# stephaneguindon/phyml

Hardware: AMD Instinct MI355X
Metric: M partial-lk site-updates/sec on full-tree Lk() (higher is better)
Workload: dtype f64

## Files before the change

### include/phyhip.h

```cpp
#ifndef PHYHIP_H
#define PHYHIP_H

#ifdef __cplusplus
extern "C" {
#endif

#define PHYHIP_SUCCESS                         0
#define PHYHIP_ERROR_GENERAL                  (-1)
#define PHYHIP_ERROR_OUT_OF_MEMORY            (-2)
#define PHYHIP_ERROR_UNIDENTIFIED_EXCEPTION   (-3)
#define PHYHIP_ERROR_UNINITIALIZED_INSTANCE   (-4)
#define PHYHIP_ERROR_OUT_OF_RANGE             (-5)
#define PHYHIP_ERROR_NO_RESOURCE              (-6)
#define PHYHIP_ERROR_NO_IMPLEMENTATION        (-7)
#define PHYHIP_ERROR_FLOATING_POINT           (-8)

#define PHYHIP_OP_NONE (-1)

#define PHYHIP_FLAG_SHARDED (1L << 40)
#define PHYHIP_UNIQUE_ID_BYTES 128
#define PHYHIP_FLAG_CLASS_AXIS (1L << 41)
#define PHYHIP_FLAG_GENERIC_LOOP (1L << 42)

typedef struct
// ... 175 lines not shown
int phyhip_get_resident_stats(int instance, long long out[8]);

int phyhip_get_big_resident_stats(int instance, long long out[4]);

int phyhip_set_virtual_buffers(int instance, int minOperations);

int phyhip_get_virtual_stats(int instance, long long out[4]);

int phyhip_get_deferred_stats(int instance, long long out[4]);

int phyhip_set_chained_buffers(int instance, int minOperations);

int phyhip_get_chained_stats(int instance, long long out[4]);

int phyhip_get_record_stats(int instance, long long out[12]);


typedef struct { int destination, child1, child2; } phyhip_parsimony_operation;

int phyhip_set_parsimony(int instance, int general, const int *stepMatrix);
int phyhip_update_partial_parsimony(int instance, const phyhip_parsimony_operation *ops, int count);
int phyhip_calculate_edge_parsimony(int instance, int buffer1, int buffer2, long long *outParsimony);
int phyhip_get_site_parsimony(int instance, int *outSitePars);
int phyhip_get_partial_parsimony(int instance, int bufferIndex, int *outUi, int *outPars, int *outPPars );
int phyhip_profile_read_parsimony(int instance, double *outKernelMs, int *outLaunches, double *outPatternUpdates);

typedef struct { int child1, child2, subtree; } phyhip_parsimony_candidate;
int phyhip_calculate_regraft_parsimony(int instance, const phyhip_parsimony_candidate *candidates, int count, int keepCandidate,
                                       long long *outParsimony );
int phyhip_get_regraft_site_parsimony(int instance, int *outSitePars );
// ... 60 lines not shown
```

### phyml_amd/capi.py

```python
from __future__ import annotations

import ctypes as C
import os

import numpy as np

_HERE = os.path.dirname(os.path.abspath(__file__))
LIB_DIR = os.environ.get("PHYHIP_LIBDIR") or os.path.join(_HERE, "lib")
LIB_PATH = os.path.join(LIB_DIR, "libphyhip.so")


class PhyhipError(RuntimeError):
    code = None


class Operation(C.Structure):
    _fields_ = [("destinationPartials", C.c_int), ("destinationScaleWrite", C.c_int), ("destinationScaleRead", C.c_int),
                ("child1Partials", C.c_int), ("child1TransitionMatrix", C.c_int),
                ("child2Partials", C.c_int), ("child2TransitionMatrix", C.c_int)]


class RegraftCandidate(C.Structure):
    _fields_ = [("child1Partials", C.c_int), ("child2Partials", C.c_int), ("subtreePartials", C.c_int), ("flags", C.c_int),
                ("child1Length", C.c_double), ("child2Length", C.c_double), ("subtreeLength", C.c_double)]
# ... 20 lines not shown
                ("flags", C.c_long), ("computeUnits", C.c_int), ("globalMemBytes", C.c_longlong)]


SYMBOLS = [
    "phyhip_create_instance", "phyhip_finalize_instance", "phyhip_get_last_error", "phyhip_set_tip_partials",
    "phyhip_set_tip_states", "phyhip_set_tip_partials_at_pattern", "phyhip_set_partials", "phyhip_set_pattern_weights", "phyhip_set_category_rates",
    "phyhip_set_category_weights", "phyhip_set_state_frequencies", "phyhip_set_eigen_decomposition",
    "phyhip_set_phyml_options", "phyhip_set_invariant_sites", "phyhip_update_transition_matrices",
    "phyhip_set_transition_matrix", "phyhip_get_transition_matrix", "phyhip_update_partials",
    "phyhip_calculate_edge_log_likelihoods", "phyhip_calculate_edge_log_likelihoods_device",
    "phyhip_get_site_log_likelihoods", "phyhip_get_site_outputs", "phyhip_get_partials", "phyhip_get_scale_factors",
    "phyhip_set_scale_factors", "phyhip_get_numerical_warning", "phyhip_update_eigen_lr",
    "phyhip_calculate_eigen_lnl_dlnl", "phyhip_calculate_eigen_lnl", "phyhip_get_dot_prod", "phyhip_set_stream",
    "phyhip_synchronize", "phyhip_profile", "phyhip_profile_read", "phyhip_calculate_mixture_log_likelihood",
    "phyhip_calculate_mixture_eigen_lnl_dlnl", "phyhip_comm_get_unique_id", "phyhip_comm_init_rank", "phyhip_comm_size",
    "phyhip_get_shard_range", "phyhip_profile_read_kernel", "phyhip_profile_read_collective", "phyhip_profile_read_traffic", "phyhip_profile_read_eigen", "phyhip_get_resident_stats", "phyhip_get_big_resident_stats", "phyhip_set_virtual_buffers", "phyhip_get_virtual_stats", "phyhip_get_deferred_stats", "phyhip_set_chained_buffers", "phyhip_get_chained_stats", "phyhip_get_record_stats", "phyhip_calculate_class_mixture_log_likelihood",
    "phyhip_calculate_class_mixture_eigen_lnl_dlnl", "phyhip_get_class_scale_factors", "phyhip_set_mixture_invariant_sites",
    "phyhip_calculate_edge_site_outputs_exact", "phyhip_calculate_node_state_posteriors", "phyhip_profile_read_node_posteriors",
    "phyhip_calculate_pairwise_ml_distances", "phyhip_set_pairwise_work_space", "phyhip_profile_read_pairwise",
    "phyhip_set_support_site_log_likelihoods", "phyhip_calculate_sh_support", "phyhip_get_support_alias_table", "phyhip_profile_read_support",
    "phyhip_set_parsimony", "phyhip_update_partial_parsimony", "phyhip_calculate_edge_parsimony", "phyhip_get_site_parsimony",
    "phyhip_get_partial_parsimony", "phyhip_profile_read_parsimony",
    "phyhip_calculate_regraft_parsimony", "phyhip_get_regraft_site_parsimony", "phyhip_get_regraft_partial_parsimony",
    "phyhip_profile_read_regraft_parsimony",
    "phyhip_optimise_edge_length", "phyhip_profile_read_edge_length",
    "phyhip_calculate_regraft_log_likelihoods", "phyhip_get_regraft_partials", "phyhip_get_regraft_transition_matrix",
    "phyhip_set_regraft_work_space", "phyhip_profile_read_regraft",
    "phyhip_calculate_mixture_regraft_log_likelihoods", "phyhip_get_mixture_regraft_partials",
    "phyhip_get_mixture_regraft_transition_matrix", "phyhip_set_mixture_regraft_work_space", "phyhip_profile_read_mixture_regraft",
    "phyhip_optimise_triples", "phyhip_get_triple_partials", "phyhip_set_triple_work_space", "phyhip_profile_read_triples",
]
# ... 68 lines not shown
def comm_get_unique_id() -> bytes:
    buf = C.create_string_buffer(UNIQUE_ID_BYTES)
    _chk(load().phyhip_comm_get_unique_id(buf))
    return buf.raw


def load():
    global _lib
    if _lib is None:
        if not os.path.exists(LIB_PATH):
            raise PhyhipError(f"{LIB_PATH} not built: run __graft_entry__.build() (hipcc --offload-arch=gfx950)")
        L = C.CDLL(LIB_PATH)
        L.phyhip_get_last_error.restype = C.c_char_p
        _lib = L
    return _lib


def _chk(rc):
    if rc < 0:
        e = PhyhipError(f"phyhip error {rc}: {load().phyhip_get_last_error().decode()}")
        e.code = rc
        raise e
    return rc


def _f64(a):
    return np.ascontiguousarray(a, dtype=np.float64)


def _ptr(a):
# ... 443 lines not shown
        return tuple(int(v) for v in out)

    def set_chained_buffers(self, min_operations):
        _chk(self.L.phyhip_set_chained_buffers(self.id, int(min_operations)))

    def chained_stats(self):
        out = (C.c_longlong * 4)()
        _chk(self.L.phyhip_get_chained_stats(self.id, out))
        return tuple(int(v) for v in out)

    def record_stats(self):
        out = (C.c_longlong * 12)()
        _chk(self.L.phyhip_get_record_stats(self.id, out))
        return tuple(int(v) for v in out)

    def profile_read_eigen(self):
        a = C.c_double(0); an = C.c_int(0); b = C.c_double(0); bn = C.c_int(0)
        _chk(self.L.phyhip_profile_read_eigen(self.id, C.byref(a), C.byref(an), C.byref(b), C.byref(bn)))
        return (a.value, an.value), (b.value, bn.value)

    def profile_read_collective(self):
        ms = C.c_double(0); n = C.c_int(0); r = C.c_int(0)
        _chk(self.L.phyhip_profile_read_collective(self.id, C.byref(ms), C.byref(n), C.byref(r)))
        return ms.value, n.value, r.value

    def profile_read_kernel(self):
        buf = C.create_string_buffer(128)
        _chk(self.L.phyhip_profile_read_kernel(self.id, buf, 128))
        return buf.value.decode()

# ... 58 lines not shown
```

### phyml_amd/csrc/phyhip.hip

```cpp
#include "phyhip_host.hpp"
#include "phyhip_side.hpp"

namespace phyhip_host
{

int fail(int code, const char *fmt, ...)
{
  char    buf[512];
  va_list ap;
  va_start(ap, fmt);
  vsnprintf(buf, sizeof buf, fmt, ap);
  va_end(ap);
  g_err = buf;
  return code;
}

}

using namespace phyhip_host;

extern "C" {

const char *phyhip_get_last_error(void) { return g_err.c_str(); }

// ... 204 lines not shown
    HIPCHK(hipMalloc((void **)&I->d_afrag, fb));
    HIPCHK(hipMemset(I->d_afrag, 0, fb));
    const long long ntiles = I->Ppad / (16 / aa_cb(I->C));
    const long long cus    = prop.multiProcessorCount > 0 ? prop.multiProcessorCount : 256;
    I->aa_nw = (int)std::min<long long>(kAaMaxCons, std::max<long long>(1, (ntiles + cus - 1) / cus));
    if (const char *e = diag_env("PHYHIP_AA_NW")) { const int v = atoi(e); if (v >= 1 && v <= kAaMaxCons) I->aa_nw = v; }
    I->aa_d2 = false;
    if (const char *e = diag_env("PHYHIP_AA_D2")) I->aa_d2 = atoi(e) != 0 && I->aa_nw <= kAaMaxConsD2;
    I->aa_nt = 1;
    if (const char *e = diag_env("PHYHIP_AA_NT")) { const int v = atoi(e); if (v == 1 || v == 2) I->aa_nt = v; }
    if (I->aa_nt == 2) I->aa_nw = std::min(I->aa_nw, 2 * kAaMaxCons2);
    I->grid_aa = (int)((ntiles + I->aa_nw - 1) / I->aa_nw);
  }
  HIPCHK(hipMalloc((void **)&I->d_tipcodes, (size_t)I->tips * I->Ppad));
  HIPCHK(hipMemset(I->d_tipcodes, 0, (size_t)I->tips * I->Ppad));
  if (I->perm)
  {
    HIPCHK(hipMalloc((void **)&I->d_tipmasks, (size_t)I->tips * I->Ppad * sizeof(uint32_t)));
    HIPCHK(hipMemset(I->d_tipmasks, 0, (size_t)I->tips * I->Ppad * sizeof(uint32_t)));
  }
  HIPCHK(hipMalloc((void **)&I->d_masks, 256 * sizeof(uint32_t)));
  HIPCHK(hipMalloc((void **)&I->d_pmats, (size_t)I->nmat_all * I->C * I->S * I->S * sizeof(double)));
  HIPCHK(hipMemset(I->d_pmats, 0, (size_t)I->nmat_all * I->C * I->S * I->S * sizeof(double)));
  HIPCHK(hipMalloc((void **)&I->d_wght, I->P * sizeof(double)));
  HIPCHK(hipMalloc((void **)&I->d_invar, I->P * sizeof(short)));
  HIPCHK(hipMemset(I->d_invar, 0xff, I->P * sizeof(short)));
  {
    std::vector<double> ones((size_t)I->P, 1.0);
    HIPCHK(hipMemcpy(I->d_wght, ones.data(), I->P * sizeof(double), hipMemcpyHostToDevice));
  }
// ... 140 lines not shown
  {
    forget_group(instance);
    release_group(G);
    return PHYHIP_SUCCESS;
  }
  GET_INST(I, instance);
  (void)hipStreamSynchronize(I->stream);
  collect_profile(I);
  (void)InstanceTable::remove(instance);
  if (I->co) release_collective(I->co);
  release_instance(I);
  return PHYHIP_SUCCESS;
}


static int set_tip_codes(Instance *I, int tip, const std::vector<uint8_t> &codes)
{
  int rc = flush(I, nullptr);
  if (rc) return rc;
  devirtualise_tip(I, tip);
  if ((rc = flush_sync(I))) return rc;
  HIPCHK(hipMemcpy(I->d_tipcodes + (size_t)tip * I->Ppad, codes.data(), (size_t)I->P, hipMemcpyHostToDevice));
  if (I->d_tipmasks)
  {
    std::vector<uint32_t> m((size_t)I->P);
    for (long long p = 0; p < I->P; ++p) m[(size_t)p] = I->masks[codes[(size_t)p]];
    HIPCHK(hipMemcpy(I->d_tipmasks + (size_t)tip * I->Ppad, m.data(), (size_t)I->P * sizeof(uint32_t), hipMemcpyHostToDevice));
  }
  return upload_masks(I);
}

static int code_for_mask(Instance *I, uint32_t m, int *code)
{
  if (m == 0) return fail(PHYHIP_ERROR_OUT_OF_RANGE, "a tip vector with no state allowed (all zeros)");
  auto it = I->mask_code.find(m);
  if (it != I->mask_code.end())
  {
// ... 53 lines not shown
  {
    const double x = inPartials[s];
    if (x == 1.0) m |= 1u << s;
    else if (x != 0.0) return fail(PHYHIP_ERROR_OUT_OF_RANGE, "tip %d pattern %d state %d: partial %g is not 0 or 1", tipIndex, pattern, s, x);
  }
  int code = (int)m;
  int rc   = 0;
  if (I->S > 8 && (rc = code_for_mask(I, m, &code))) return rc;
  if ((rc = flush(I, nullptr))) return rc;
  devirtualise_tip(I, tipIndex);
  if ((rc = flush(I, nullptr))) return rc;
  void *st = nullptr;
  if ((rc = I->ring.alloc(16, I->stream, &st))) return rc;
  *reinterpret_cast<uint8_t *>(st) = (uint8_t)code;
  *(reinterpret_cast<uint32_t *>(st) + 1) = m;
  I->stream_dirty = true; I->touched_call = true;
  HIPCHK(hipMemcpyAsync(I->d_tipcodes + (size_t)tipIndex * I->Ppad + pattern, st, 1, hipMemcpyHostToDevice, I->stream));
  if (I->d_tipmasks)
    HIPCHK(hipMemcpyAsync(I->d_tipmasks + (size_t)tipIndex * I->Ppad + pattern, reinterpret_cast<uint32_t *>(st) + 1, 4,
                          hipMemcpyHostToDevice, I->stream));
  return upload_masks(I);
}

int phyhip_set_tip_states(int instance, int tipIndex, const int *inStates)
{
  if (Group *G = get_group(instance))
    return group_each(G, [&](int id, long long lo, long long) { return phyhip_set_tip_states(id, tipIndex, inStates + lo); });
  GET_INST(I, instance);
  if (tipIndex < 0 || tipIndex >= I->tips) return fail(PHYHIP_ERROR_OUT_OF_RANGE, "tip index %d", tipIndex);
  std::vector<uint8_t> codes((size_t)I->P);
// ... 740 lines not shown
  if (Group *G = get_group(instance)) return phyhip_get_chained_stats(G->sub_id[0], out);
  GET_INST(I, instance);
  const Unstored::Counters &c = I->unstored.counters(Unstored::kChained);
  out[0] = I->unstored.n(Unstored::kChained); out[1] = (long long)c.skipped; out[2] = (long long)c.material; out[3] = (long long)c.dropped;
  return PHYHIP_SUCCESS;
}

int phyhip_get_record_stats(int instance, long long out[12])
{
  if (Group *G = get_group(instance)) return phyhip_get_record_stats(G->sub_id[0], out);
  GET_INST(I, instance);
  memcpy(out, I->rec_stats, sizeof I->rec_stats);
  return PHYHIP_SUCCESS;
}

int phyhip_profile_read_collective(int instance, double *outMs, int *outCount, int *outRanks)
{
  Group *G = get_group(instance);
  GET_INST(I, G ? G->sub_id[0] : instance);
  int rc = flush_sync(I);
  if (rc) return rc;
  if ((rc = collect_profile(I))) return rc;
  if (outMs) *outMs = I->prof_aux_ms[2];
  if (outCount) *outCount = I->prof_aux_n[2];
  const Collective *co = G ? G->co : I->co;
  if (outRanks) *outRanks = co ? co->nranks : 1;
  return PHYHIP_SUCCESS;
}

int phyhip_profile_read_kernel(int instance, char *outName, int capacity)
// ... 32 lines not shown
```

### phyml_amd/csrc/phyhip_host.hpp

```cpp
#pragma once
#include "../../include/phyhip.h"
#include "phyhip_kernels.hpp"
#include "phyhip_aa.hpp"
#include "phyhip_nt2.hpp"
#include "phyhip_big.hpp"
#include "phyhip_matrix_queue.hpp"

#include <rccl/rccl.h>

#include <cfloat>
#include <functional>
#include <cmath>
#include <cstdarg>
#include <cstdio>
#include <cstdlib>
#include <cstring>
#include <ctime>
#include <atomic>
#include <chrono>
#include <condition_variable>
#include <mutex>
#include <thread>
#include <string>
#include <unordered_map>
// ... 267 lines not shown
  unsigned long long clean_epoch = 0, rt_epoch = 0;
  bool         touched_call = false;
  bool               stream_dirty = true, dirty_prev = true;
  unsigned long long stamp_seq = 0, clean_after = 0;
  unsigned long long model_epoch = 1;
  unsigned long long api_no = 0, eig_api_no = 0;
  bool               fenced_eval = false;
  int          wall_khz = 0;
  bool      host_sum   = true;
  void     *d_pmscratch = nullptr;
  int       pm_scratch_cap = 0;
  char     *d_ops      = nullptr;
  size_t    ops_slot_bytes = 0;
  int       ops_cap = 0, ops_slots = 4, ops_slot = 0;
  long long rec_stats[12] = {0};
  int       grid = 0, grid_nt = 0, block_nt = 64;

  std::vector<DevOp>                     pending;
  Unstored                               unstored;
  bool                                   virt_inline = true;
  std::vector<InlineDef>                 pending_inl;
  std::vector<std::vector<InlineDef>>    slot_inl;
  MatrixTable<double>                    rebuilds;
  MatrixTable<const double *>            uploads;
  std::vector<unsigned char>             mat_in_queue;
  std::vector<std::vector<DevOp>>        slot_ops;
  std::vector<int>                       slot_kind;
  std::vector<uint32_t>                  masks;
  std::unordered_map<uint32_t, int>      mask_code;
  bool                                   masks_dirty = false;
// ... 208 lines not shown
int  flush_pmats(Instance *I);
bool fuse_reduce(const Instance *I, int nblocks);
int  flush(Instance *I, const EdgeEval *ee);
int  flush_sync(Instance *I);
int  flush_and_wait(Instance *I, EdgeEval &ee, bool flushed = false);
int  check_partial_index(const Instance *I, int idx, bool allow_tip);
int  wait_host_sum(Instance *I);
int  wait_result(Instance *I);
int  collect_profile(Instance *I);

constexpr int kOpNoStore = 1;
constexpr int kOpInl1 = 2, kOpInl2 = 4;
void devirtualise(Instance *I, int buf);
void devirtualise_all(Instance *I);
void devirtualise_matrix(Instance *I, int m);
void devirtualise_tip(Instance *I, int tip);
void devirtualise_dependants(Instance *I, int buf);
inline int shadow_slot(const Instance *I, int b, int w) { return I->nmat + 2 * (b - I->tips) + w; }
void rewrite_pending(Instance *I, const EdgeEval *ee, bool may_virtualise);

constexpr int kResidentMaxGrid = 64;
inline bool dlk_from_len(const Instance *I) { return I->S == 20 && I->NE == 1 && !I->class_axis && I->C <= 8; }
constexpr int kResidentSilent = -4242;
static double ns_since(const struct timespec &t0)
{
  struct timespec t1;
  clock_gettime(CLOCK_MONOTONIC, &t1);
  return (double)(t1.tv_sec - t0.tv_sec) * 1e9 + (double)(t1.tv_nsec - t0.tv_nsec);
}

// ... 103 lines not shown
```

### phyml_amd/csrc/phyhip_kernels.hpp

```cpp
#pragma once

#include <hip/hip_runtime.h>
#include <stdint.h>

#include "phyhip_exp.hpp"
#include "phyhip_log.hpp"

namespace phyhip
{

typedef const __attribute__((address_space(3))) unsigned long long *ExpLdsTab;
#ifdef PHYHIP_OCML_EXP
__device__ __forceinline__ double dev_exp(const double x, const unsigned long long * = nullptr) { return exp(x); }
#else
__device__ __forceinline__ double dev_exp(const double x) { return phyhip_exp_ref(x, phyhip_exp_tab); }
__device__ __forceinline__ double dev_exp(const double x, const unsigned long long *lds)
{
  return lds ? phyhip_exp_ref(x, (ExpLdsTab)lds) : phyhip_exp_ref(x, phyhip_exp_tab);
}
#endif
__device__ __forceinline__ void exp_tab_to_lds(unsigned long long *lds, const int tid, const int nth)
{
  for (int i = tid; i < 256; i += nth) lds[i] = phyhip_exp_tab[i];
}
// ... 59 lines not shown
struct alignas(16) NtExec
{
  unsigned fl;
  unsigned dst_data;
  unsigned dst_scale;
  unsigned pad;
};
enum : unsigned
{
  kRecL1 = 1u, kRecL2 = 2u,
  kRecA1 = 4u, kRecA2 = 8u,
  kRecT1 = 16u, kRecT2 = 32u,
  kRecIn1 = 64u, kRecIn2 = 128u,
  kRecStore = 256u
};

struct TreeParams
{
  double         *partials;
  int            *scales;
  const double   *wght;
  long long       P;
  long long       Ppad;
  int             perm;
  int             C;
  int             tip_count;
  int             apply_scaling;
  int             n_ops;
  int             last_dest;
  int             edge_eval;
// ... 1726 lines not shown
```

### phyml_amd/csrc/phyhip_nt2.hpp

```cpp
#pragma once
#ifndef PHYHIP_LOAD_AUX
#define PHYHIP_LOAD_AUX 2
#endif
#ifndef PHYHIP_STORE_AUX
#define PHYHIP_STORE_AUX 2
#endif

#include "phyhip_kernels.hpp"

namespace phyhip
{

typedef unsigned int u32x2 __attribute__((ext_vector_type(2)));

struct NtFresh
{
  const int    *idx;
  const double *len;
  const double *evec, *ivec, *eval, *rates;
  const int    *up_idx = nullptr;
  const double *up_val = nullptr;
  bool          up_sys = false;
  const unsigned long long *exp_lds = nullptr;
};

template <int C, int G, bool DBG, int ARGS, int DIST = 2, int NW = 1, bool LREC = false, bool INL = false>
__device__ __forceinline__ void nt2_run(const TreeParams &q, const IssueRec *__restrict__ irec, const ExecRec *__restrict__ xrec,
                                        const double *pmats,
                                        const uint8_t *__restrict__ tip_codes, unsigned long long *dbg, const NtFresh fr,
                                        const unsigned tile, const unsigned tid, double *lds_dot, const unsigned rec_no = 0xffffffffu)
{
  __shared__ unsigned long long stamps[DBG ? 64 * 8 : 1];
  const bool stamper = DBG && tile == gridDim.x / 2 && tid == 0;
#define PHY_STAMP(k_, i_)                                                                                              \
  if (DBG)                                                                                                             \
  {                                                                                                                    \
    const unsigned long long t_ = __builtin_readcyclecounter();                                                        \
    if (stamper && (k_) < 64) stamps[(k_) * 8 + (i_)] = t_;                                                            \
  }
  static_assert(C % G == 0 && 64 % G == 0, "category groups must divide the categories and the wave");
  constexpr int S = 4, CL = C / G, CS = CL * S, PW = 64 / G;
// ... 377 lines not shown
          if constexpr (G > 1)
          {
            if (!cls) mx = group_max(mx);
          }
          if (mx < kHiInvTwoToLarge && q.apply_scaling)
          {
#pragma unroll
            for (int e = 0; e < CS; ++e) XC[e] *= kTwoToLarge;
            scx = kLarge;
          }
        }
      };
      const unsigned tcx = INL ? ((R.tx >> tsh) & 255u) : 0u;
      bool in1 = false, in2 = false;
      if constexpr (INL) { in1 = (fl & kOpCh1) != 0; in2 = (fl & kOpCh2) != 0; }
      if constexpr (INL)
      {
        if (in1)
        {
          cherry(tca, tcx);
          matvec_x(buf, XC, u1);
          s1 = scx; one1 = (XC[0] == 1.0);
        }
      }
      if (in1) {}
      else if (fl & kOpTip1)
      {
        tip_u(bufd, buf, tca, u1);
        s1 = 0; one1 = (tca == 15u);
      }
// ... 9 lines not shown
          matvec_x(buf + C * 8, XC, u2);
          s2 = scx; one2 = (XC[0] == 1.0);
        }
      }
      if (in2) {}
      else if (fl & kOpTip2)
      {
        tip_u(bufd + C * 16, buf + C * 8, tcb, u2);
        s2 = 0; one2 = (tcb == 15u);
      }
      else if (fl & kOpF21) { matvec_x(buf + C * 8, Fprev, u2); s2 = scprev; one2 = (Fprev[0] == 1.0); }
      else if (fl & kOpF22) { matvec_x(buf + C * 8, Fout, u2); s2 = scout; one2 = (Fout[0] == 1.0); }
      else { matvec_r(buf + C * 8, R.b, u2); s2 = R.sb; one2 = (first_d(R.b[0]) == 1.0); }

      PHY_STAMP(k, 2)
      unsigned ones_mask = 0;
      if (__builtin_amdgcn_ballot_w64(one1 && one2))
      {
        double ra[CS], rb[CS];
        unpack(R.a, ra);
        unpack(R.b, rb);
#pragma unroll
        for (int c = 0; c < CL; ++c)
        {
          bool a1, a2;
          if (fl & kOpTip1) a1 = (tca == 15u);
          else
          {
            a1 = true;
#pragma unroll
            for (int j = 0; j < S; ++j)
              a1 = a1 && ((in1 ? XC[INL ? c * 4 + j : 0] : (fl & kOpF11) ? Fprev[c * 4 + j] : (fl & kOpF12) ? Fout[c * 4 + j] : ra[c * 4 + j]) == 1.0);
          }
          if (fl & kOpTip2) a2 = (tcb == 15u);
          else
          {
            a2 = true;
#pragma unroll
            for (int j = 0; j < S; ++j)
              a2 = a2 && ((in2 ? XC[INL ? c * 4 + j : 0] : (fl & kOpF21) ? Fprev[c * 4 + j] : (fl & kOpF22) ? Fout[c * 4 + j] : rb[c * 4 + j]) == 1.0);
          }
          ones_mask |= (a1 && a2) ? (1u << c) : 0u;
        }
      }

      PHY_STAMP(k, 3)
      IRec nx3;
      if constexpr (early)
      {
        __builtin_amdgcn_sched_barrier(0);
        __builtin_amdgcn_s_waitcnt(0xc07f);
        nx1 = XR((k + 1 < last) ? k + 1 : last);
        stage_pm(parity ^ 1, PN, PN2);
        __builtin_amdgcn_sched_barrier(0);
      }
      if constexpr (!ARGS) issue(nx2, R, PC, PC2);
      PHY_STAMP(k, 7)
      nx3 = IR((k + 1 + DIST < last) ? k + 1 + DIST : last);
      if constexpr (early) __builtin_amdgcn_sched_barrier(0);
      __builtin_amdgcn_wave_barrier();
      PHY_STAMP(k, 4)

      unsigned mxh = 0;
#pragma unroll
      for (int e = 0; e < CS; ++e)
      {
        const double v = ((ones_mask >> (e / 4)) & 1u) ? 1.0 : u1[e] * u2[e];
        Fout[e] = v;
        mxh     = max(mxh, hi32(v));
      }
      if constexpr (G > 1)
      {
        if (!cls) mxh = group_max(mxh);
      }
      unsigned sc = s1 + s2;
      if (mxh < kHiInvTwoToLarge && q.apply_scaling)
      {
#pragma unroll
        for (int e = 0; e < CS; ++e) Fout[e] *= kTwoToLarge;
        sc += kLarge;
      }
      scout = sc;
      PHY_STAMP(k, 5)
      {
// ... 198 lines not shown
                                                             const uint8_t *__restrict__ tip_codes,
                                                             unsigned long long *dbg = nullptr)
{
  typedef const __attribute__((address_space(4))) char karg_char;
  const char *ka = (const char *)(karg_char *)__builtin_amdgcn_kernarg_segment_ptr();
  NtFresh     fr;
  fr.idx  = reinterpret_cast<const int *>(ka + offsetof(TreeParams, fresh_idx));
  fr.len  = reinterpret_cast<const double *>(ka + offsetof(TreeParams, fresh_len));
  fr.evec = reinterpret_cast<const double *>(ka + offsetof(TreeParams, m_evec));
  fr.ivec = reinterpret_cast<const double *>(ka + offsetof(TreeParams, m_ivec));
  fr.eval = reinterpret_cast<const double *>(ka + offsetof(TreeParams, m_eval));
  fr.rates = reinterpret_cast<const double *>(ka + offsetof(TreeParams, m_rates));
  fr.up_idx = reinterpret_cast<const int *>(ka + offsetof(TreeParams, up_idx));
  fr.up_val = reinterpret_cast<const double *>(ka + offsetof(TreeParams, up_val));
  __shared__ __attribute__((aligned(16))) double lds_dot[(64 / G) * C * 4];
  nt2_run<C, G, DBG, ARGS, DIST, 1, false, INL>(q, irec, xrec, pmats, tip_codes, dbg, fr, blockIdx.x, threadIdx.x, lds_dot);
}

template <int C, bool INL>
__global__ __launch_bounds__(64, 2) void traverse_nt2_mixed_kernel(const TreeParams q, const IssueRec *__restrict__ irec,
                                                                   const ExecRec *__restrict__ xrec, const double *pmats,
                                                                   const uint8_t *__restrict__ tip_codes, const int n2)
{
  static_assert(C == 4, "four-lane waves: one category per lane");
  typedef const __attribute__((address_space(4))) char karg_char;
  const char *ka = (const char *)(karg_char *)__builtin_amdgcn_kernarg_segment_ptr();
  NtFresh     fr;
  fr.idx  = reinterpret_cast<const int *>(ka + offsetof(TreeParams, fresh_idx));
  fr.len  = reinterpret_cast<const double *>(ka + offsetof(TreeParams, fresh_len));
  fr.evec = reinterpret_cast<const double *>(ka + offsetof(TreeParams, m_evec));
  fr.ivec = reinterpret_cast<const double *>(ka + offsetof(TreeParams, m_ivec));
  fr.eval = reinterpret_cast<const double *>(ka + offsetof(TreeParams, m_eval));
  fr.rates = reinterpret_cast<const double *>(ka + offsetof(TreeParams, m_rates));
  fr.up_idx = reinterpret_cast<const int *>(ka + offsetof(TreeParams, up_idx));
  fr.up_val = reinterpret_cast<const double *>(ka + offsetof(TreeParams, up_val));
  __shared__ __attribute__((aligned(16))) double lds_dot[32 * C * 4];
  if ((int)blockIdx.x < n2)
    nt2_run<C, 2, false, 0, 2, 1, false, INL>(q, irec, xrec, pmats, tip_codes, nullptr, fr, blockIdx.x, threadIdx.x, lds_dot);
  else
    nt2_run<C, 4, false, 0, 2, 1, false, INL>(q, irec, xrec, pmats, tip_codes, nullptr, fr, 2u * (unsigned)n2 + (blockIdx.x - (unsigned)n2),
                                              threadIdx.x, lds_dot, blockIdx.x);
}

constexpr int kResidentNtWords = 10 + 2 * 12;

template <int C, int G>
__global__ __launch_bounds__(64, 1) void resident_nt2_kernel(const TreeParams sq, const ResidentCtl r, const double *pmats,
                                                             const uint8_t *__restrict__ tip_codes, const double *evec,
                                                             const double *ivec, const double *eval, const double *rates)
{
  __shared__ unsigned long long sh_raw[64];
  __shared__ int                sh_idx[4];
  __shared__ double             sh_len[4];
  __shared__ __attribute__((aligned(16))) double sh_dot[(64 / G) * C * 4];
  __shared__ unsigned long long sh_exp[256];
// ... 57 lines not shown
```

### phyml_amd/csrc/phyhip_queue.hip

```cpp
#include "phyhip_host.hpp"
#include <algorithm>

namespace phyhip_host
{

int flush_uploads(Instance *I)
{
  const auto &up = I->uploads;
  if (!up.empty())
  {
    big_release(I);
    I->touched_call = true;
  }
  size_t done = 0;
  while (done < up.size())
  {
    const int n = (int)std::min<size_t>(up.size() - done, kUploadBatch);
    MatUploadParams q;
    memset(&q, 0, sizeof q);
    q.count = n; q.S = I->S; q.C = I->C; q.pmats = I->d_pmats; q.afrag = I->perm ? I->d_afrag : nullptr;
    for (int k = 0; k < kUploadBatch; ++k) q.shadow[k] = -1;
    for (int k = 0; k < n; ++k) { q.idx[k] = up.idx()[done + k]; q.src[k] = up.payload()[done + k]; q.shadow[k] = up.snapshot()[done + k]; }
    hipLaunchKernelGGL(upload_matrices_kernel, dim3(n), dim3(256), q.afrag ? sizeof(double) * (size_t)I->C * I->S * I->S : 0, I->stream, q);
    HIPCHK(hipGetLastError());
// ... 292 lines not shown
  if (!I->soa || I->perm) return false;
  const int g = I->nt_groups;
  return (I->C == 1 && g == 1) || (I->C == 2 && g <= 2) || (I->C == 3 && g == 1) || (I->C == 4 && (g == 1 || g == 2 || g == 4));
}

static int fill_compact_records(Instance *I, const FlushPlan &f, NtIssue *ir, NtExec *xr, int n_rec)
{
  const int    n_ops = f.n_ops;
  const size_t data16 = buf_elems(I) * sizeof(double) / 16, scale16 = scale_elems(I) * 4 / 16, tip16 = (size_t)I->Ppad / 16;
  const size_t n_int = (size_t)(I->nbuf - I->tips);
  if (n_int * data16 > 0xffffffffull || (size_t)I->tips * tip16 > 0xffffffffull || I->tips >= (1 << 24))
    return fail(PHYHIP_ERROR_OUT_OF_RANGE, "an arena of this instance is beyond the reach of a record's offset (64 GiB, 2^24 tips)");
  const unsigned matbytes = (unsigned)((size_t)I->C * I->S * I->S * sizeof(double));
  auto at = [&](int k) -> const DevOp & { return I->pending[std::min(k, n_ops - 1)]; };
  long long (&kinds)[2][5] = *reinterpret_cast<long long (*)[2][5]>(I->rec_stats + 2);
  ++I->rec_stats[0];
  for (int k = 0; k < n_rec; ++k)
  {
    const DevOp     &o  = at(k);
    const int        e1 = k >= 1 ? at(k - 1).dest : -1;
    const int        e2 = (k >= 2 && I->prefetch_dist == 2) ? at(k - 2).dest : -1;
    const InlineDef *inl = (o.pad & (kOpInl1 | kOpInl2)) ? &I->pending_inl[std::min(k, n_ops - 1)] : nullptr;
    NtIssue          r;
    memset(&r, 0, sizeof r);
    unsigned fl = 0;
    auto child = [&](int c, int s, int pm, bool in_step) {
      r.pm[s] = (unsigned)pm * matbytes;
      if (in_step)
      {
        r.fl |= (kRecIn1 | kRecA1 | kRecT1) << s | (unsigned)inl->b << 8;
        r.data[s] = (unsigned)inl->pmA * matbytes; r.pmx = (unsigned)inl->pmB * matbytes;
        r.aux[s] = (unsigned)((size_t)inl->a * tip16);
        fl |= kOpCh1 << s;
        ++kinds[s][1];
        return;
      }
      const size_t b = (size_t)(c - I->tips);
      if (c < I->tips) { r.fl |= (kRecA1 | kRecT1) << s; r.aux[s] = (unsigned)((size_t)c * tip16); fl |= kOpTip1 << s; ++kinds[s][0]; }
      else if (c == e1) { fl |= s ? kOpF21 : kOpF11; ++kinds[s][2]; }
      else if (c == e2) { fl |= s ? kOpF22 : kOpF12; ++kinds[s][3]; }
      else
      {
        if (!I->no_loads) { r.fl |= (kRecL1 | kRecA1) << s; r.data[s] = (unsigned)(b * data16); r.aux[s] = (unsigned)(b * scale16); }
        ++kinds[s][4];
      }
    };
    child(o.c1, 0, o.pm1, inl && (o.pad & kOpInl1));
    child(o.c2, 1, o.pm2, inl && (o.pad & kOpInl2));
    ir[k] = r;
    const size_t b = (size_t)(o.dest - I->tips);
    xr[k].fl = fl | ((o.pad & kOpNoStore) ? 0u : kRecStore);
    xr[k].dst_data = (unsigned)(b * data16); xr[k].dst_scale = (unsigned)(b * scale16); xr[k].pad = 0;
  }
  return 0;
}

static int build_op_records(Instance *I, FlushPlan &f, TreeParams &q)
{
  const int  n_ops = f.n_ops;
  const bool fat = f.fat;
  q.last_dest = -1;
  if (n_ops == 0) return 0;
  const bool   compact = fat && compact_list_form(I) && !f.big_cmd();
  const int    kind = fat ? (compact ? 16 : 0) + I->prefetch_dist : 0, n_rec = n_ops + (n_ops & 1);
  const size_t ib = (compact ? sizeof(NtIssue) : sizeof(IssueRec)) * n_rec, xb = (compact ? sizeof(NtExec) : sizeof(ExecRec)) * n_rec;
  int          hit = -1, rc = 0;
  for (int sl = 0; sl < I->ops_slots && hit < 0; ++sl)
// ... 314 lines not shown
{
  if (I->prof) snprintf(I->prof_kernel, sizeof I->prof_kernel, fmt, a...);
}

template <typename K> static void launch_nt2_form(K kernel, Instance *I, const FlushPlan &f, const TreeParams &q, unsigned long long *dbg = nullptr)
{
  hipLaunchKernelGGL(kernel, dim3(I->grid_nt2), dim3(64), 0, I->stream, q, f.d_irec, f.d_xrec, f.ro.pmats, f.ro.tip_codes, dbg);
}
template <typename K> static void launch_aa_form(K kernel, Instance *I, dim3 blk, const FlushPlan &f, const TreeParams &q, unsigned long long *dbg = nullptr)
{
  hipLaunchKernelGGL(kernel, dim3(I->grid_aa), blk, 0, I->stream, q, f.d_irec, f.d_xrec, (const double *)I->d_afrag, I->nmat_all,
                     (const uint32_t *)I->d_tipmasks, dbg, AaResident());
}

#ifdef PHYHIP_DIAG
static int print_stamps(Instance *I, int n_steps, bool load_issue, int &printed)
{
  if (printed++ != 5) return 0;
  unsigned long long h[64 * 8];
  HIPCHK(hipMemcpyAsync(h, I->d_dbg, sizeof h, hipMemcpyDeviceToHost, I->stream));
  HIPCHK(hipStreamSynchronize(I->stream));
  for (int k = 0; k < 64 && k < n_steps; ++k)
  {
    fprintf(stderr, "step %2d:", k);
    for (int i = 1; i < 7; ++i) fprintf(stderr, " %6lld", (long long)(h[k * 8 + i] - h[k * 8 + i - 1]));
    if (k + 1 < 64) fprintf(stderr, "  | next %6lld", (long long)(h[(k + 1) * 8] - h[k * 8 + 6]));
    if (load_issue) fprintf(stderr, "  | load issue %6lld of segment 4", (long long)(h[k * 8 + 7] - h[k * 8 + 3]));
    fprintf(stderr, "\n");
  }
  return 0;
}

static int launch_nt2_diag(Instance *I, const FlushPlan &f, const TreeParams &q)
{
  if (!((I->ablate & 8) && I->C == 4 && I->nt_groups <= 2)) return kNotLaunched;
  if (!I->d_dbg) HIPCHK(hipMalloc((void **)&I->d_dbg, 64 * 8 * 8));
  if (I->nt_groups == 2) launch_nt2_form(traverse_nt2_kernel<4, 2, true>, I, f, q, I->d_dbg);
  else launch_nt2_form(traverse_nt2_kernel<4, 1, true>, I, f, q, I->d_dbg);
  static int printed = 0;
  return print_stamps(I, q.n_ops, true, printed);
}

static int launch_aa_diag(Instance *I, dim3 blk, const FlushPlan &f, const TreeParams &q)
{
  if (I->C == 4 && I->ablate >= 256)
  {
#define AAABL(a_) case a_: launch_aa_form(traverse_aa_kernel<4, false, a_>, I, blk, f, q); return 0;
    switch (I->ablate - 256)
    {
      AAABL(1) AAABL(2) AAABL(4) AAABL(8) AAABL(9) AAABL(16) AAABL(18) AAABL(5) AAABL(13) AAABL(31) AAABL(27)
      default: break;
    }
#undef AAABL
  }
  if (!((I->ablate & 8) && I->ablate < 256 && I->C == 4)) return kNotLaunched;
// ... 128 lines not shown
      if (I->perm)
        if (const int rc = launch_perm(I, f, q); rc != kNotLaunched) return rc;
    named(I, "traverse_kernel<%d, %d>", S_, CP_);
    hipLaunchKernelGGL((traverse_kernel<S_, CP_>), dim3(I->grid), dim3(256), 0, I->stream, q, f.ro.ops, f.ro.pmats, f.ro.tip_codes,
                       f.ro.code_masks);
    return 0;
  });
}

static int flush_impl(Instance *I, const EdgeEval *ee)
{
  const unsigned long long hp0 = hp_now();
  FlushPlan f;
  f.n_queued = (int)I->pending.size();
  rewrite_pending(I, ee, (I->soa || I->perm) && !I->generic_nt && I->prefetch_dist == 2 && !I->class_axis && !I->generic_loop &&
                             !I->ablate && !I->no_loads);
  I->unstored.keep_clear();
  const int n_ops = f.n_ops = (int)I->pending.size();
  int       rc = 0;
  if (n_ops > 0 || ee || !I->rebuilds.empty() || !I->uploads.empty()) I->stream_dirty = true;
  if (ee) I->fenced_eval = false;
  if ((rc = plan_route(I, ee, f))) return rc;
  if (!f.fold_pm && !f.up_ride && (!I->rebuilds.empty() || !I->uploads.empty()) && (rc = flush_pmats(I))) return rc;
  if (n_ops == 0 && !ee) return 0;
  if ((rc = upload_masks(I))) return rc;

  TreeParams q = base_params(I);
  f.ro      = base_ro(I, nullptr);
  f.fat     = ((I->S == 4) && !I->generic_nt) || I->perm;
  f.has_inl = !I->pending_inl.empty();
  fill_matrix_args(I, f, q);
// ... 254 lines not shown
```

Before: 49460.

## Add specialized step bodies for one-hot tip and forwarded children in nt2 kernel

Tracks per-tip host statistics (ambiguous-code and all-gap counts) to classify each traversal step by child kind: unambiguous tip, forwarded from the previous step, or in-step pair. The kind is encoded in the exec record flags. The kernel then dispatches to compile-time specialized bodies that read a single matrix column for one-hot tips and skip the generic loading and ones-mask path. This is meant to cut loads and FLOPs for tip-heavy steps. In exchange it adds host bookkeeping on tip updates, more register pressure and code size in the kernel, and a wave-wide ballot fallback when forwarded partials equal one.

Measured after the change: 53530 (median of 6 runs). +8.2%, better.

```diff
diff --git a/include/phyhip.h b/include/phyhip.h
--- a/include/phyhip.h
+++ b/include/phyhip.h
@@ -213,6 +213,10 @@
 int phyhip_get_chained_stats(int instance, long long out[4]);
 
 int phyhip_get_record_stats(int instance, long long out[12]);
+
+int phyhip_get_step_kind_stats(int instance, long long out[16]);
+
+int phyhip_tip_row_bits(const unsigned char *codes, long long n);
 
 
 typedef struct { int destination, child1, child2; } phyhip_parsimony_operation;
diff --git a/phyml_amd/capi.py b/phyml_amd/capi.py
--- a/phyml_amd/capi.py
+++ b/phyml_amd/capi.py
@@ -58,7 +58,7 @@
     "phyhip_calculate_eigen_lnl_dlnl", "phyhip_calculate_eigen_lnl", "phyhip_get_dot_prod", "phyhip_set_stream",
     "phyhip_synchronize", "phyhip_profile", "phyhip_profile_read", "phyhip_calculate_mixture_log_likelihood",
     "phyhip_calculate_mixture_eigen_lnl_dlnl", "phyhip_comm_get_unique_id", "phyhip_comm_init_rank", "phyhip_comm_size",
-    "phyhip_get_shard_range", "phyhip_profile_read_kernel", "phyhip_profile_read_collective", "phyhip_profile_read_traffic", "phyhip_profile_read_eigen", "phyhip_get_resident_stats", "phyhip_get_big_resident_stats", "phyhip_set_virtual_buffers", "phyhip_get_virtual_stats", "phyhip_get_deferred_stats", "phyhip_set_chained_buffers", "phyhip_get_chained_stats", "phyhip_get_record_stats", "phyhip_calculate_class_mixture_log_likelihood",
+    "phyhip_get_shard_range", "phyhip_profile_read_kernel", "phyhip_profile_read_collective", "phyhip_profile_read_traffic", "phyhip_profile_read_eigen", "phyhip_get_resident_stats", "phyhip_get_big_resident_stats", "phyhip_set_virtual_buffers", "phyhip_get_virtual_stats", "phyhip_get_deferred_stats", "phyhip_set_chained_buffers", "phyhip_get_chained_stats", "phyhip_get_record_stats", "phyhip_get_step_kind_stats", "phyhip_tip_row_bits", "phyhip_calculate_class_mixture_log_likelihood",
     "phyhip_calculate_class_mixture_eigen_lnl_dlnl", "phyhip_get_class_scale_factors", "phyhip_set_mixture_invariant_sites",
     "phyhip_calculate_edge_site_outputs_exact", "phyhip_calculate_node_state_posteriors", "phyhip_profile_read_node_posteriors",
     "phyhip_calculate_pairwise_ml_distances", "phyhip_set_pairwise_work_space", "phyhip_profile_read_pairwise",
@@ -157,6 +157,11 @@
         L.phyhip_get_last_error.restype = C.c_char_p
         _lib = L
     return _lib
+
+
+def tip_row_bits(codes):
+    a = np.ascontiguousarray(codes, dtype=np.uint8)
+    return int(load().phyhip_tip_row_bits(a.ctypes.data_as(C.c_void_p), C.c_longlong(a.size)))
 
 
 def _chk(rc):
@@ -630,6 +635,11 @@
         _chk(self.L.phyhip_get_record_stats(self.id, out))
         return tuple(int(v) for v in out)
 
+    def step_kind_stats(self):
+        out = (C.c_longlong * 16)()
+        _chk(self.L.phyhip_get_step_kind_stats(self.id, out))
+        return tuple(int(v) for v in out[:8]), tuple(int(v) for v in out[8:])
+
     def profile_read_eigen(self):
         a = C.c_double(0); an = C.c_int(0); b = C.c_double(0); bn = C.c_int(0)
         _chk(self.L.phyhip_profile_read_eigen(self.id, C.byref(a), C.byref(an), C.byref(b), C.byref(bn)))
diff --git a/phyml_amd/csrc/phyhip.hip b/phyml_amd/csrc/phyhip.hip
--- a/phyml_amd/csrc/phyhip.hip
+++ b/phyml_amd/csrc/phyhip.hip
@@ -242,6 +242,12 @@
   }
   HIPCHK(hipMalloc((void **)&I->d_tipcodes, (size_t)I->tips * I->Ppad));
   HIPCHK(hipMemset(I->d_tipcodes, 0, (size_t)I->tips * I->Ppad));
+  if (I->S == 4)
+  {
+    I->h_tiprows.assign((size_t)I->tips * I->P, 0);
+    I->tip_namb.assign((size_t)I->tips, I->P);
+    I->tip_n15.assign((size_t)I->tips, 0);
+  }
   if (I->perm)
   {
     HIPCHK(hipMalloc((void **)&I->d_tipmasks, (size_t)I->tips * I->Ppad * sizeof(uint32_t)));
@@ -412,6 +418,33 @@
 }
 
 
+static bool tip_code_ambiguous(unsigned m) { return !(m == 1u || m == 2u || m == 4u || m == 8u); }
+static void tip_row_counts(const unsigned char *codes, long long n, long long &namb, long long &n15)
+{
+  namb = n15 = 0;
+  for (long long p = 0; p < n; ++p)
+  {
+    namb += tip_code_ambiguous(codes[p]);
+    n15 += codes[p] == 15u;
+  }
+}
+static int tip_bits_of(long long namb, long long n15) { return (namb == 0 ? 1 : 0) | (n15 != 0 ? 2 : 0); }
+int phyhip_tip_row_bits(const unsigned char *codes, long long n)
+{
+  long long namb, n15;
+  tip_row_counts(codes, n, namb, n15);
+  return tip_bits_of(namb, n15);
+}
+
+static int tip_bits_now(const Instance *I, int tip) { return tip_bits_of(I->tip_namb[(size_t)tip], I->tip_n15[(size_t)tip]); }
+static void tip_bits_changed(Instance *I, int tip, int before)
+{
+  if (tip_bits_now(I, tip) == before) return;
+  for (int &k : I->slot_kind)
+    if (k >= 16) k = -1;
+}
+extern "C++" int phyhip_host::tip_row_bits(const Instance *I, int tip) { return I->h_tiprows.empty() ? 0 : tip_bits_now(I, tip); }
+
 static int set_tip_codes(Instance *I, int tip, const std::vector<uint8_t> &codes)
 {
   int rc = flush(I, nullptr);
@@ -419,6 +452,13 @@
   devirtualise_tip(I, tip);
   if ((rc = flush_sync(I))) return rc;
   HIPCHK(hipMemcpy(I->d_tipcodes + (size_t)tip * I->Ppad, codes.data(), (size_t)I->P, hipMemcpyHostToDevice));
+  if (!I->h_tiprows.empty())
+  {
+    const int before = tip_bits_now(I, tip);
+    memcpy(I->h_tiprows.data() + (size_t)tip * I->P, codes.data(), (size_t)I->P);
+    tip_row_counts(codes.data(), I->P, I->tip_namb[(size_t)tip], I->tip_n15[(size_t)tip]);
+    tip_bits_changed(I, tip, before);
+  }
   if (I->d_tipmasks)
   {
     std::vector<uint32_t> m((size_t)I->P);
@@ -502,6 +542,15 @@
   if ((rc = I->ring.alloc(16, I->stream, &st))) return rc;
   *reinterpret_cast<uint8_t *>(st) = (uint8_t)code;
   *(reinterpret_cast<uint32_t *>(st) + 1) = m;
+  if (!I->h_tiprows.empty())
+  {
+    const int before = tip_bits_now(I, tipIndex);
+    uint8_t  &was = I->h_tiprows[(size_t)tipIndex * I->P + pattern];
+    I->tip_namb[(size_t)tipIndex] += (long long)tip_code_ambiguous((unsigned)code) - (long long)tip_code_ambiguous(was);
+    I->tip_n15[(size_t)tipIndex] += (long long)(code == 15) - (long long)(was == 15);
+    was = (uint8_t)code;
+    tip_bits_changed(I, tipIndex, before);
+  }
   I->stream_dirty = true; I->touched_call = true;
   HIPCHK(hipMemcpyAsync(I->d_tipcodes + (size_t)tipIndex * I->Ppad + pattern, st, 1, hipMemcpyHostToDevice, I->stream));
   if (I->d_tipmasks)
@@ -1272,6 +1321,15 @@
   return PHYHIP_SUCCESS;
 }
 
+int phyhip_get_step_kind_stats(int instance, long long out[2 * 8])
+{
+  if (Group *G = get_group(instance)) return phyhip_get_step_kind_stats(G->sub_id[0], out);
+  GET_INST(I, instance);
+  static_assert(kNtStepKinds == 8, "out[2][8]");
+  memcpy(out, I->step_kinds, sizeof I->step_kinds);
+  return PHYHIP_SUCCESS;
+}
+
 int phyhip_profile_read_collective(int instance, double *outMs, int *outCount, int *outRanks)
 {
   Group *G = get_group(instance);
diff --git a/phyml_amd/csrc/phyhip_host.hpp b/phyml_amd/csrc/phyhip_host.hpp
--- a/phyml_amd/csrc/phyhip_host.hpp
+++ b/phyml_amd/csrc/phyhip_host.hpp
@@ -305,6 +305,10 @@
   size_t    ops_slot_bytes = 0;
   int       ops_cap = 0, ops_slots = 4, ops_slot = 0;
   long long rec_stats[12] = {0};
+  long long step_kinds[2][kNtStepKinds] = {{0}};
+  std::vector<uint8_t>   h_tiprows;
+  std::vector<long long> tip_namb, tip_n15;
+  std::vector<unsigned>  last_exec_fl;
   int       grid = 0, grid_nt = 0, block_nt = 64;
 
   std::vector<DevOp>                     pending;
@@ -543,6 +547,7 @@
 void devirtualise(Instance *I, int buf);
 void devirtualise_all(Instance *I);
 void devirtualise_matrix(Instance *I, int m);
+int  tip_row_bits(const Instance *I, int tip);
 void devirtualise_tip(Instance *I, int tip);
 void devirtualise_dependants(Instance *I, int buf);
 inline int shadow_slot(const Instance *I, int b, int w) { return I->nmat + 2 * (b - I->tips) + w; }
diff --git a/phyml_amd/csrc/phyhip_kernels.hpp b/phyml_amd/csrc/phyhip_kernels.hpp
--- a/phyml_amd/csrc/phyhip_kernels.hpp
+++ b/phyml_amd/csrc/phyhip_kernels.hpp
@@ -97,6 +97,12 @@
   kRecIn1 = 64u, kRecIn2 = 128u,
   kRecStore = 256u
 };
+constexpr unsigned kRecKindShift = 12u;
+constexpr int      kNtStepKinds  = 8;
+#ifndef PHYHIP_NT_KINDS
+#define PHYHIP_NT_KINDS 0x7e
+#endif
+constexpr bool nt2_bodied(int C, int G, bool INL) { return G >= 2 && !(C == 4 && G == 2 && !INL) && !(C == 2 && G == 2 && INL); }
 
 struct TreeParams
 {
diff --git a/phyml_amd/csrc/phyhip_nt2.hpp b/phyml_amd/csrc/phyhip_nt2.hpp
--- a/phyml_amd/csrc/phyhip_nt2.hpp
+++ b/phyml_amd/csrc/phyhip_nt2.hpp
@@ -24,7 +24,7 @@
   const unsigned long long *exp_lds = nullptr;
 };
 
-template <int C, int G, bool DBG, int ARGS, int DIST = 2, int NW = 1, bool LREC = false, bool INL = false>
+template <int C, int G, bool DBG, int ARGS, int DIST = 2, int NW = 1, bool LREC = false, bool INL = false, bool BODIES = false>
 __device__ __forceinline__ void nt2_run(const TreeParams &q, const IssueRec *__restrict__ irec, const ExecRec *__restrict__ xrec,
                                         const double *pmats,
                                         const uint8_t *__restrict__ tip_codes, unsigned long long *dbg, const NtFresh fr,
@@ -432,6 +432,110 @@
       const unsigned tcx = INL ? ((R.tx >> tsh) & 255u) : 0u;
       bool in1 = false, in2 = false;
       if constexpr (INL) { in1 = (fl & kOpCh1) != 0; in2 = (fl & kOpCh2) != 0; }
+      unsigned ones_mask = 0;
+      bool     ones_any = false;
+      constexpr bool bodied = BODIES && compact && G >= 2 && DIST == 2;
+      bool fast = false;
+      if constexpr (bodied)
+      {
+        auto col = [&](const double *Md, const unsigned m, double (&u)[CS]) {
+          const int s = (m >> 1) - (m >> 3);
+#pragma unroll
+          for (int e = 0; e < CS; ++e) u[e] = Md[(c0 * S + e) * 4 + s];
+        };
+        auto rows = [&](const double2 *M, double2 (&m)[CL * 8]) {
+#pragma unroll
+          for (int i = 0; i < CL * 8; ++i) m[i] = M[c0 * 8 + i];
+        };
+        auto matvec_m = [&](const double2 (&m)[CL * 8], const double (&x)[CS], double (&u)[CS]) {
+#pragma unroll
+          for (int c = 0; c < CL; ++c)
+#pragma unroll
+            for (int i = 0; i < S; ++i)
+            {
+              const double2 lo = m[c * 8 + 2 * i], hi = m[c * 8 + 2 * i + 1];
+              double        a  = lo.x * x[c * 4];
+              a = __builtin_fma(lo.y, x[c * 4 + 1], a);
+              a = __builtin_fma(hi.x, x[c * 4 + 2], a);
+              a = __builtin_fma(hi.y, x[c * 4 + 3], a);
+              u[c * 4 + i] = a;
+            }
+        };
+        auto body = [&](auto k1_, auto k2_) {
+          constexpr int K1 = decltype(k1_)::value, K2 = decltype(k2_)::value;
+          constexpr int PI = (K1 == 2) ? 0 : 1, PO = 1 - PI;
+          constexpr int KO = (K1 == 2) ? K2 : (K2 == 2) ? K1 : -1;
+          if constexpr (K1 + K2 == 3)
+          {
+            if (__builtin_amdgcn_ballot_w64(Fprev[0] == 1.0) != 0) return;
+          }
+          fast = true;
+          if constexpr (K1 != 2 && K2 != 2)
+          {
+            constexpr int PT = (K1 == 0) ? 0 : 1;
+            double2       mf[CL * 8];
+            double (&ut)[CS] = PT == 0 ? u1 : u2;
+            double (&uf)[CS] = PT == 0 ? u2 : u1;
+            col(bufd + PT * C * 16, PT == 0 ? tca : tcb, ut);
+            rows(buf + (1 - PT) * C * 8, mf);
+            matvec_m(mf, Fprev, uf);
+            (PT == 0 ? s1 : s2) = 0;
+            (PT == 0 ? s2 : s1) = scprev;
+          }
+          else if constexpr (INL)
+          {
+            double  ua[CS], ub[CS];
+            double2 mo[CL * 8], mi[CL * 8];
+            double (&ui)[CS] = PI == 0 ? u1 : u2;
+            double (&uo)[CS] = PI == 0 ? u2 : u1;
+            col(bufd + 2 * C * 16, PI == 0 ? tca : tcb, ua);
+            col(bufd + 3 * C * 16, tcx, ub);
+            if constexpr (KO == 0) col(bufd + PO * C * 16, PO == 0 ? tca : tcb, uo);
+            else rows(buf + PO * C * 8, mo);
+            unsigned mx = 0;
+#pragma unroll
+            for (int e = 0; e < CS; ++e)
+            {
+              XC[e] = ua[e] * ub[e];
+              mx    = max(mx, hi32(XC[e]));
+            }
+            if constexpr (KO == 1) matvec_m(mo, Fprev, uo);
+            if constexpr (G > 1)
+            {
+              if (!cls) mx = group_max(mx);
+            }
+            if (mx < kHiInvTwoToLarge && q.apply_scaling)
+            {
+#pragma unroll
+              for (int e = 0; e < CS; ++e) XC[e] *= kTwoToLarge;
+              scx = kLarge;
+            }
+            rows(buf + PI * C * 8, mi);
+            matvec_m(mi, XC, ui);
+            (PI == 0 ? s1 : s2) = scx;
+            (PI == 0 ? s2 : s1) = KO == 0 ? 0u : scprev;
+          }
+        };
+        using std::integral_constant;
+        constexpr unsigned on = PHYHIP_NT_KINDS;
+        switch ((fl >> kRecKindShift) & 7u)
+        {
+          case 1: if constexpr ((on >> 1) & 1) body(integral_constant<int, 0>(), integral_constant<int, 1>()); break;
+          case 2: if constexpr ((on >> 2) & 1) body(integral_constant<int, 1>(), integral_constant<int, 0>()); break;
+          case 3: if constexpr (INL && ((on >> 3) & 1)) body(integral_constant<int, 2>(), integral_constant<int, 1>()); break;
+          case 4: if constexpr (INL && ((on >> 4) & 1)) body(integral_constant<int, 1>(), integral_constant<int, 2>()); break;
+          case 5: if constexpr (INL && ((on >> 5) & 1)) body(integral_constant<int, 2>(), integral_constant<int, 0>()); break;
+          case 6: if constexpr (INL && ((on >> 6) & 1)) body(integral_constant<int, 0>(), integral_constant<int, 2>()); break;
+          default: break;
+        }
+      }
+      if (fast)
+      {
+        PHY_STAMP(k, 1)
+        PHY_STAMP(k, 2)
+      }
+      else
+      {
       if constexpr (INL)
       {
         if (in1)
@@ -471,8 +575,8 @@
       else { matvec_r(buf + C * 8, R.b, u2); s2 = R.sb; one2 = (first_d(R.b[0]) == 1.0); }
 
       PHY_STAMP(k, 2)
-      unsigned ones_mask = 0;
-      if (__builtin_amdgcn_ballot_w64(one1 && one2))
+      ones_any = __builtin_amdgcn_ballot_w64(one1 && one2) != 0;
+      if (ones_any)
       {
         double ra[CS], rb[CS];
         unpack(R.a, ra);
@@ -501,6 +605,7 @@
         }
       }
 
+      }
       PHY_STAMP(k, 3)
       IRec nx3;
       if constexpr (early)
@@ -519,12 +624,24 @@
       PHY_STAMP(k, 4)
 
       unsigned mxh = 0;
-#pragma unroll
-      for (int e = 0; e < CS; ++e)
-      {
-        const double v = ((ones_mask >> (e / 4)) & 1u) ? 1.0 : u1[e] * u2[e];
-        Fout[e] = v;
-        mxh     = max(mxh, hi32(v));
+      if (bodied && !ones_any)
+      {
+#pragma unroll
+        for (int e = 0; e < CS; ++e)
+        {
+          Fout[e] = u1[e] * u2[e];
+          mxh     = max(mxh, hi32(Fout[e]));
+        }
+      }
+      else
+      {
+#pragma unroll
+        for (int e = 0; e < CS; ++e)
+        {
+          const double v = ((ones_mask >> (e / 4)) & 1u) ? 1.0 : u1[e] * u2[e];
+          Fout[e] = v;
+          mxh     = max(mxh, hi32(v));
+        }
       }
       if constexpr (G > 1)
       {
@@ -753,7 +870,7 @@
   fr.up_idx = reinterpret_cast<const int *>(ka + offsetof(TreeParams, up_idx));
   fr.up_val = reinterpret_cast<const double *>(ka + offsetof(TreeParams, up_val));
   __shared__ __attribute__((aligned(16))) double lds_dot[(64 / G) * C * 4];
-  nt2_run<C, G, DBG, ARGS, DIST, 1, false, INL>(q, irec, xrec, pmats, tip_codes, dbg, fr, blockIdx.x, threadIdx.x, lds_dot);
+  nt2_run<C, G, DBG, ARGS, DIST, 1, false, INL, ARGS == 0 && DIST == 2 && nt2_bodied(C, G, INL)>(q, irec, xrec, pmats, tip_codes, dbg, fr, blockIdx.x, threadIdx.x, lds_dot);
 }
 
 template <int C, bool INL>
@@ -775,9 +892,9 @@
   fr.up_val = reinterpret_cast<const double *>(ka + offsetof(TreeParams, up_val));
   __shared__ __attribute__((aligned(16))) double lds_dot[32 * C * 4];
   if ((int)blockIdx.x < n2)
-    nt2_run<C, 2, false, 0, 2, 1, false, INL>(q, irec, xrec, pmats, tip_codes, nullptr, fr, blockIdx.x, threadIdx.x, lds_dot);
+    nt2_run<C, 2, false, 0, 2, 1, false, INL, true>(q, irec, xrec, pmats, tip_codes, nullptr, fr, blockIdx.x, threadIdx.x, lds_dot);
   else
-    nt2_run<C, 4, false, 0, 2, 1, false, INL>(q, irec, xrec, pmats, tip_codes, nullptr, fr, 2u * (unsigned)n2 + (blockIdx.x - (unsigned)n2),
+    nt2_run<C, 4, false, 0, 2, 1, false, INL, true>(q, irec, xrec, pmats, tip_codes, nullptr, fr, 2u * (unsigned)n2 + (blockIdx.x - (unsigned)n2),
                                               threadIdx.x, lds_dot, blockIdx.x);
 }
 
diff --git a/phyml_amd/csrc/phyhip_queue.hip b/phyml_amd/csrc/phyhip_queue.hip
--- a/phyml_amd/csrc/phyhip_queue.hip
+++ b/phyml_amd/csrc/phyhip_queue.hip
@@ -330,6 +330,8 @@
   const unsigned matbytes = (unsigned)((size_t)I->C * I->S * I->S * sizeof(double));
   auto at = [&](int k) -> const DevOp & { return I->pending[std::min(k, n_ops - 1)]; };
   long long (&kinds)[2][5] = *reinterpret_cast<long long (*)[2][5]>(I->rec_stats + 2);
+  const bool mixed  = I->mix_n4 > 0 && I->C == 4 && I->nt_groups == 2 && !I->ablate;
+  const bool bodied = I->prefetch_dist == 2 && I->nt_groups >= 2 && (mixed || nt2_bodied(I->C, I->nt_groups, f.has_inl));
   ++I->rec_stats[0];
   for (int k = 0; k < n_rec; ++k)
   {
@@ -340,10 +342,13 @@
     NtIssue          r;
     memset(&r, 0, sizeof r);
     unsigned fl = 0;
+    int      how[2] = {-1, -1};
+    auto     onehot = [&](int tip) { return (tip_row_bits(I, tip) & 1) != 0; };
     auto child = [&](int c, int s, int pm, bool in_step) {
       r.pm[s] = (unsigned)pm * matbytes;
       if (in_step)
       {
+        if (onehot(inl->a) && onehot(inl->b)) how[s] = 2;
         r.fl |= (kRecIn1 | kRecA1 | kRecT1) << s | (unsigned)inl->b << 8;
         r.data[s] = (unsigned)inl->pmA * matbytes; r.pmx = (unsigned)inl->pmB * matbytes;
         r.aux[s] = (unsigned)((size_t)inl->a * tip16);
@@ -352,8 +357,8 @@
         return;
       }
       const size_t b = (size_t)(c - I->tips);
-      if (c < I->tips) { r.fl |= (kRecA1 | kRecT1) << s; r.aux[s] = (unsigned)((size_t)c * tip16); fl |= kOpTip1 << s; ++kinds[s][0]; }
-      else if (c == e1) { fl |= s ? kOpF21 : kOpF11; ++kinds[s][2]; }
+      if (c < I->tips) { r.fl |= (kRecA1 | kRecT1) << s; r.aux[s] = (unsigned)((size_t)c * tip16); fl |= kOpTip1 << s; ++kinds[s][0]; if (onehot(c)) how[s] = 0; }
+      else if (c == e1) { fl |= s ? kOpF21 : kOpF11; ++kinds[s][2]; how[s] = 1; }
       else if (c == e2) { fl |= s ? kOpF22 : kOpF12; ++kinds[s][3]; }
       else
       {
@@ -364,9 +369,15 @@
     child(o.c1, 0, o.pm1, inl && (o.pad & kOpInl1));
     child(o.c2, 1, o.pm2, inl && (o.pad & kOpInl2));
     ir[k] = r;
+    static const unsigned char kind_of[3][3] = {{0, 1, 6}, {2, 0, 4}, {5, 3, 0}};
+    unsigned kind = (how[0] >= 0 && how[1] >= 0) ? kind_of[how[0]][how[1]] : 0u;
+    if (!((PHYHIP_NT_KINDS >> kind) & 1) || !bodied) kind = 0;
+    ++I->step_kinds[k & 1][kind];
+    fl |= kind << kRecKindShift;
     const size_t b = (size_t)(o.dest - I->tips);
     xr[k].fl = fl | ((o.pad & kOpNoStore) ? 0u : kRecStore);
     xr[k].dst_data = (unsigned)(b * data16); xr[k].dst_scale = (unsigned)(b * scale16); xr[k].pad = 0;
+    if (kDiag) { I->last_exec_fl.resize((size_t)n_rec); I->last_exec_fl[(size_t)k] = xr[k].fl; }
   }
   return 0;
 }
@@ -711,7 +722,7 @@
 }
 
 #ifdef PHYHIP_DIAG
-static int print_stamps(Instance *I, int n_steps, bool load_issue, int &printed)
+static int print_stamps(Instance *I, int n_steps, bool load_issue, int &printed, const std::vector<unsigned> *fl = nullptr)
 {
   if (printed++ != 5) return 0;
   unsigned long long h[64 * 8];
@@ -723,6 +734,12 @@
     for (int i = 1; i < 7; ++i) fprintf(stderr, " %6lld", (long long)(h[k * 8 + i] - h[k * 8 + i - 1]));
     if (k + 1 < 64) fprintf(stderr, "  | next %6lld", (long long)(h[(k + 1) * 8] - h[k * 8 + 6]));
     if (load_issue) fprintf(stderr, "  | load issue %6lld of segment 4", (long long)(h[k * 8 + 7] - h[k * 8 + 3]));
+    if (fl && k < (int)fl->size())
+    {
+      const unsigned x = (*fl)[(size_t)k];
+      auto           how = [&](int s) { return (x & (kOpCh1 << s)) ? "in-step" : (x & (kOpTip1 << s)) ? "tip" : (x & (s ? kOpF21 : kOpF11)) ? "fwd1" : (x & (s ? kOpF22 : kOpF12)) ? "fwd2" : "loaded"; };
+      fprintf(stderr, "  | kind %u: %s x %s%s", (x >> kRecKindShift) & 7u, how(0), how(1), (x & kRecStore) ? ", stored" : "");
+    }
     fprintf(stderr, "\n");
   }
   return 0;
@@ -732,10 +749,12 @@
 {
   if (!((I->ablate & 8) && I->C == 4 && I->nt_groups <= 2)) return kNotLaunched;
   if (!I->d_dbg) HIPCHK(hipMalloc((void **)&I->d_dbg, 64 * 8 * 8));
-  if (I->nt_groups == 2) launch_nt2_form(traverse_nt2_kernel<4, 2, true>, I, f, q, I->d_dbg);
+  if (I->nt_groups == 2 && f.has_inl) launch_nt2_form(traverse_nt2_kernel<4, 2, true, 0, 2, true>, I, f, q, I->d_dbg);
+  else if (f.has_inl) return fail(PHYHIP_ERROR_NO_IMPLEMENTATION, "PHYHIP_ABLATE=8: the stamped form with in-step children is the two-lane one");
+  else if (I->nt_groups == 2) launch_nt2_form(traverse_nt2_kernel<4, 2, true>, I, f, q, I->d_dbg);
   else launch_nt2_form(traverse_nt2_kernel<4, 1, true>, I, f, q, I->d_dbg);
   static int printed = 0;
-  return print_stamps(I, q.n_ops, true, printed);
+  return print_stamps(I, q.n_ops, true, printed, &I->last_exec_fl);
 }
 
 static int launch_aa_diag(Instance *I, dim3 blk, const FlushPlan &f, const TreeParams &q)
@@ -894,7 +913,7 @@
   FlushPlan f;
   f.n_queued = (int)I->pending.size();
   rewrite_pending(I, ee, (I->soa || I->perm) && !I->generic_nt && I->prefetch_dist == 2 && !I->class_axis && !I->generic_loop &&
-                             !I->ablate && !I->no_loads);
+                             !(I->ablate & ~8) && !I->no_loads);
   I->unstored.keep_clear();
   const int n_ops = f.n_ops = (int)I->pending.size();
   int       rc = 0;
```
